# mumianyuxin/M3DSSD

Hardware: AMD Instinct MI355X
Metric: images/sec at 1280x384 bs=8, 1/2/4/8 MI355X; 3D-box Linf vs ref (higher is better)
Workload: dtype f32; 1 GPU; BASELINE.json configs[1]: full M3d_inference_align (DLA-34 + DCNv2 align + ANAB) forward + decode + top-3000 + NMS, bs=8/GPU, 1280x384, fp32, random-init synthetic weights and frames; per_gpu_batch=8, global_batch=8, parallelism=dp1 (batch sharded, 1 all-gather of [B,40,14] detections)

## Files before the change

### include/m3dssd_hip.h

```cpp
#ifndef M3DSSD_HIP_H
#define M3DSSD_HIP_H

#include <stdint.h>

#ifdef __cplusplus
extern "C" {
#endif

typedef void *m3d_stream_t;

enum {
    M3D_OK = 0,
    M3D_E_ARG = -1,
    M3D_E_HIP = -2,
    M3D_E_WORKSPACE = -3
};

const char *m3d_last_error(void);
#define M3D_ABI_VERSION 5
int m3d_abi_version(void);
const char *m3d_source_hashes(void);

typedef struct m3d_conv_desc {
    const float *in;
// ... 9 lines not shown
    int out_nchw;
    long long out_img_stride;
    const float *scale;
    const float *shift;
    const float *res;
    int res_cs;
    int res_mode;
    int act;
    int sigmoid_from;
    const float *dcn_offmask;
    int dcn_om_cs;
    float *splitk_ws;
    long long splitk_ws_bytes;
} m3d_conv_desc;

int m3d_conv2d_forward(const m3d_conv_desc *d, m3d_stream_t stream);
int m3d_conv2d_splitk_plan(const m3d_conv_desc *d, int *splits, long long *ws_bytes);

int m3d_conv_wave_applicable(const m3d_conv_desc *d);
int m3d_conv_wave_splitk_plan(const m3d_conv_desc *d, int *splits, long long *ws_bytes);
int m3d_conv_wave_forward(const m3d_conv_desc *d, m3d_stream_t stream);
int m3d_conv_wave_forward_wgsplit(const m3d_conv_desc *d, m3d_stream_t stream);
int m3d_conv_wave_wgsplit_width(const m3d_conv_desc *d, int *slices, int *width);

int m3d_wino_conv3x3_forward(const m3d_conv_desc *d, m3d_stream_t stream);
int m3d_wino_conv3x3_variant(const m3d_conv_desc *d);
int m3d_wino_conv3x3_splitk_plan(const m3d_conv_desc *d, int *splits, long long *ws_bytes);
int m3d_wino_conv3x3_forward_ex(const m3d_conv_desc *d, int variant, m3d_stream_t stream);
int m3d_wino44_applicable(const m3d_conv_desc *d);
int m3d_wino44_conv3x3_forward(const m3d_conv_desc *d, m3d_stream_t stream);
int m3d_wino44_conv3x3_forward_ex(const m3d_conv_desc *d, int nb, m3d_stream_t stream);
int m3d_wino44_kpair(const m3d_conv_desc *d);
int m3d_wino44_splitk_plan(const m3d_conv_desc *d, int *splits, long long *ws_bytes);
int m3d_wino44_conv3x3_forward_touch(const m3d_conv_desc *d, int nb, const void *touch, long long touch_bytes, m3d_stream_t stream);

int m3d_cache_touch(const void *p, long long bytes, m3d_stream_t stream);
int m3d_upload_indirect(const void *const *src_slot, void *dst, long long bytes, m3d_stream_t stream);

int m3d_conv2d_tile(const m3d_conv_desc *d, int *bm, int *bn, int *bk, int *grid);

typedef struct m3d_conv_bf16_desc {
    const void *in;
    int in_cs;
    int N, H, W, Cin;
    const void *wgt;
    long long wgt_img_stride;
// ... 346 lines not shown
                            long long box_img_stride, m3d_stream_t stream);

int m3d_anab_pool_partial(const float *kv, int kv_cs, const float *s, int s_cs, const int *items, int n_items,
                          const int *bin_scale, int n_bins, float *partial, int max_slots, int B, int H, int W,
                          int C, m3d_stream_t stream);
int m3d_anab_pool_finish(const float *partial, const int *bin_slots, const float *bin_inv_area, int n_bins,
                         int max_slots, int Ck, int Cv, float *khat, int keys_pad, int ck_pad, float *vhatT,
                         int B, int frag, m3d_stream_t stream);
long long m3d_anab_pool_nested_scratch_bytes(int B, int C);
int m3d_anab_pool_nested(const float *kv, int kv_cs, const float *s, int s_cs, int B, int H, int W, int Ck, int Cv,
                         float *scratch, float *khat, int keys_pad, int ck_pad, float *vhatT, int frag, m3d_stream_t stream);
int m3d_anab_pool_nested_bf16(const void *kv, int kv_cs, const float *s, int s_cs, int B, int H, int W, int Ck, int Cv,
                              float *scratch, float *khat, int keys_pad, int ck_pad, float *vhatT, int frag, m3d_stream_t stream);
int m3d_anab_pool_nested_bf16_ex(const void *kv, int kv_cs, const float *s, int s_cs, int B, int H, int W, int Ck, int Cv,
                                 float *scratch, float *khat, int keys_pad, int ck_pad, float *vhatT, int frag,
                                 void *khat16, void *vhat16, m3d_stream_t stream);
int m3d_anab_attend_f32(const float *q, int q_cs, const float *khat, int k_cs, const float *vhatT, int B, int HW, int Ck,
                        int keys, int keys_pad, int Cv, const float *res, int res_cs, int res_mode, const float *scale,
                        const float *shift, int act, float *out, int out_cs, m3d_stream_t stream);
int m3d_anab_attend_f32_rows(const float *q, int q_cs, const float *khat, int k_cs, const float *vhatT, int B, int HW, int Ck,
                             int keys, int keys_pad, int Cv, const float *res, int res_cs, int res_mode, const float *scale,
                             const float *shift, int act, float *out, int out_cs, const int *rows, const int *n_rows,
                             m3d_stream_t stream);
long long m3d_anab_attention_workspace_bytes(int B, int H, int W, int Ck, int Cv, int backward);
int m3d_anab_attention_forward(const float *q, const float *k, const float *v, const float *g, float *out, int B, int H, int W, int Ck,
                               int Cv, int q_cs, int k_cs, int v_cs, int g_cs, int out_cs, void *workspace, long long workspace_bytes,
                               m3d_stream_t stream);
int m3d_anab_attention_backward(const float *q, const float *k, const float *v, const float *g, const float *grad_out, float *grad_q,
                                float *grad_k, float *grad_v, float *grad_g, int B, int H, int W, int Ck, int Cv, int q_cs, int k_cs,
                                int v_cs, int g_cs, int go_cs, int gq_cs, int gk_cs, int gv_cs, int gg_cs, void *workspace,
                                long long workspace_bytes, m3d_stream_t stream);
long long m3d_anab_attention_workspace_bytes_bf16(int B, int H, int W, int Ck, int Cv, int backward);
int m3d_anab_attention_forward_bf16(const void *q, const void *k, const void *v, const void *g, void *out, int B, int H, int W, int Ck,
                                    int Cv, int q_cs, int k_cs, int v_cs, int g_cs, int out_cs, void *workspace,
                                    long long workspace_bytes, m3d_stream_t stream);
int m3d_anab_attention_backward_bf16(const void *q, const void *k, const void *v, const void *g, const void *grad_out, void *grad_q,
                                     void *grad_k, void *grad_v, void *grad_g, int B, int H, int W, int Ck, int Cv, int q_cs, int k_cs,
                                     int v_cs, int g_cs, int go_cs, int gq_cs, int gk_cs, int gv_cs, int gg_cs, void *workspace,
                                     long long workspace_bytes, m3d_stream_t stream);
int m3d_softmax_rows(float *x, int rows, int valid, int cs, m3d_stream_t stream);

int m3d_bundle_outputs(const float *cls_planar, const float *box_planar, float *cls, float *prob, float *bbox_2d,
                       float *bbox_3d, unsigned int *score_bits, int B, int A, int HW, m3d_stream_t stream);
int m3d_score_keys_planar(const float *cls_planar, unsigned int *score_bits, int B, int A, int HW, m3d_stream_t stream);
long long m3d_topk_decode_workspace_bytes(int B, int R);
int m3d_topk_decode(const unsigned int *score_bits, const float *prob, const float *bbox_2d, const float *bbox_3d,
// ... 75 lines not shown
```

### m3dssd_amd/csrc/anab_attend.hip

```cpp
#include <stdlib.h>

#include "common.h"

#define AF_CV 128
#define AF_KT 32
#define AF_VROW (AF_KT * 4 + 16)

struct AnabF32Args {
    const float *q, *khat, *vhat, *res, *scale, *shift;
    float *out;
    int q_cs, k_cs, HW, Ck, keys, keys_pad, res_cs, out_cs, res_mode, act;
};

template <int CK, int NSPLIT>
__device__ __forceinline__ void anab_attend_f32_body(const AnabF32Args &a, const int img, const int mq, const bool store)
{
    constexpr int KROW = CK * 4 + 16;
    constexpr int NS4 = CK / 8;
    __shared__ __attribute__((aligned(16))) unsigned char lds[AF_KT * KROW + AF_CV * AF_VROW];
    unsigned char *Ks = lds, *Vs = lds + AF_KT * KROW;
    const int tid = threadIdx.x, lane = tid & 63;
    const int l31 = lane & 31, lh = lane >> 5;

    f32x4 qf[NS4];
// ... 199 lines not shown
    }
    M3D_LAUNCH_CHECK();
    return M3D_OK;
}

extern "C" int m3d_anab_attend_f32(const float *q, int q_cs, const float *khat, int k_cs, const float *vhatT, int B, int HW, int Ck,
                                   int keys, int keys_pad, int Cv, const float *res, int res_cs, int res_mode, const float *scale,
                                   const float *shift, int act, float *out, int out_cs, m3d_stream_t stream)
{
    return anab_attend_f32_launch(q, q_cs, khat, k_cs, vhatT, B, HW, Ck, keys, keys_pad, Cv, res, res_cs, res_mode, scale, shift, act,
                                  out, out_cs, nullptr, nullptr, stream);
}

extern "C" int m3d_anab_attend_f32_rows(const float *q, int q_cs, const float *khat, int k_cs, const float *vhatT, int B, int HW, int Ck,
                                        int keys, int keys_pad, int Cv, const float *res, int res_cs, int res_mode,
                                        const float *scale, const float *shift, int act, float *out, int out_cs, const int *rows,
                                        const int *n_rows, m3d_stream_t stream)
{
    M3D_REQUIRE(rows && n_rows, "anab_attend_f32_rows: null row list");
    M3D_REQUIRE((long long)B * HW < 0x7FFFFFFFLL - 64, "anab_attend_f32_rows: too many pixels");
    return anab_attend_f32_launch(q, q_cs, khat, k_cs, vhatT, B, HW, Ck, keys, keys_pad, Cv, res, res_cs, res_mode, scale, shift, act,
                                  out, out_cs, rows, n_rows, stream);
}
```

### m3dssd_amd/csrc/dcn_wave.hip

```cpp

#include <type_traits>

#include "common.h"

struct ConvWaveArgs {
    const float *in, *wfrag, *scale, *shift, *res, *om;
    float *out;
    int in_cs, out_cs, res_cs, om_cs;
    int H, W, Cin, Ho, Wo, HoWo, Cout;
    int kh, kw, stride, pad, dil;
    int M, KG, tiles_n;
    int act, res_mode, sigmoid_from;
    int vec_out;
    long long w_img_stride;
    unsigned in_bytes, out_bytes, res_bytes, w_bytes;
    float *ws;
    int splits, ss_per, base_waves;
    unsigned ws_bytes;
#ifdef CONV_TRACE
    long long *trace;
#endif
};


#ifdef CONV_TRACE
static long long *g_conv_trace = nullptr;
extern "C" void m3d_conv_wave_set_trace(void *buf) { g_conv_trace = (long long *)buf; }
static int g_conv_variant = 0;
extern "C" void m3d_conv_wave_set_variant(int v) { g_conv_variant = v; }
#define TRACE_INIT() long long *trp = (a.trace && threadIdx.x < 64) ? a.trace + (size_t)blockIdx.x * 128 : nullptr; int tri = 0
#define TRACE() do { if (trp && lane == 0 && tri < 128) trp[tri++] = __builtin_readcyclecounter(); } while (0)
#else
#define TRACE_INIT()
#define TRACE()
#endif

template <bool DEFORM, int NT, int NCQ = 4, int WPE = (DEFORM ? 2 : 3), int S = 1>
__global__ __launch_bounds__(64 * S) __attribute__((amdgpu_waves_per_eu(WPE))) void conv_wave_kernel(const ConvWaveArgs a)
{
    __shared__ __attribute__((aligned(16))) float tileS[S * 32 * 32];
    __shared__ __attribute__((aligned(16))) float tapst[(DEFORM ? 9 : 1) * 32 * 8];
    const int lane = threadIdx.x & 63, l31 = lane & 31, h = lane >> 5;
    const int wv = S > 1 ? __builtin_amdgcn_readfirstlane((int)threadIdx.x >> 6) : 0;
    float *const tileA = tileS + wv * 1024;
    const int gp = lane >> 3, gc = lane & 7;
    TRACE_INIT();
    TRACE();
    int blk;
    {
        const int nblk = gridDim.x, bid = blockIdx.x;
        const int q = nblk >> 3, r = nblk & 7, xcd = bid & 7, loc = bid >> 3;
        blk = (xcd < r ? xcd * (q + 1) : r * (q + 1) + (xcd - r) * q) + loc;
    }
    int split = wv;
    if (S == 1 && a.splits > 1) {
        split = blk / a.base_waves;
        blk -= split * a.base_waves;
    }
    const int bm = blk / a.tiles_n, bn = blk - bm * a.tiles_n;
    const int m0 = bm * 32;
    const int KK = a.kh * a.kw, C32 = a.Cin / 32;
    const bool idle = S > 1 && wv >= a.splits;
    const int ss0 = idle ? 0 : split * a.ss_per, ss1 = idle ? 0 : min(KK * C32, ss0 + a.ss_per);

    const __amdgpu_buffer_rsrc_t rin = make_rsrc(a.in, a.in_bytes);
    const __amdgpu_buffer_rsrc_t rw =
        make_rsrc(a.wfrag + (size_t)(m0 / a.HoWo) * a.w_img_stride + (size_t)bn * NT * a.KG * 256, a.w_bytes);
    const unsigned wlane = (unsigned)lane * 16u;
    const unsigned wstride = (unsigned)a.KG * 1024u;

    int o_pix = 0, o_hi0 = 0, o_wi0 = 0;
    bool o_valid = false;
    int o_inv = -1;
    const float *o_om = a.om;
    int g_pix[4], g_hi0[4], g_wi0[4];
    bool g_valid[4];
    {
        const int m = m0 + l31;
        o_valid = m < a.M;
        o_inv = sign_smear(a.M - 1 - m);
        const int mm = o_valid ? m : 0;
        const int n = mm / a.HoWo, rem = mm - n * a.HoWo;
        const int ho = rem / a.Wo, wo = rem - ho * a.Wo;
        o_pix = n * a.H * a.W;
        o_hi0 = ho * a.stride - a.pad;
        o_wi0 = wo * a.stride - a.pad;
        if (DEFORM) o_om = a.om + (size_t)mm * a.om_cs;
    }
    if constexpr (!DEFORM) {
#pragma unroll
        for (int g = 0; g < 4; ++g) {
            const int m = m0 + 8 * g + gp;
            g_valid[g] = m < a.M;
            const int mm = g_valid[g] ? m : 0;
            const int n = mm / a.HoWo, rem = mm - n * a.HoWo;
            const int ho = rem / a.Wo, wo = rem - ho * a.Wo;
            g_pix[g] = n * a.H * a.W;
            g_hi0[g] = ho * a.stride - a.pad;
            g_wi0[g] = wo * a.stride - a.pad;
        }
    }

    unsigned doff[4][DEFORM ? 4 : 1];
    float bw[DEFORM ? 4 : 1][4];
    if constexpr (DEFORM) {
        constexpr int TPW = (9 + S - 1) / S;
        float raws[TPW][3];
#pragma unroll
        for (int i = 0; i < TPW; ++i) {
            const int tp = min(wv + i * S, KK - 1);
            raws[i][0] = o_om[2 * tp];
            raws[i][1] = o_om[2 * tp + 1];
            raws[i][2] = o_om[2 * KK + tp];
        }
#pragma unroll
        for (int i = 0; i < TPW; ++i) {
            const int t = wv + i * S;
// ... 200 lines not shown
                    const float *p = &tileS[px[q] * 32 + 4 * c4];
                    f32x4 v = *reinterpret_cast<const f32x4 *>(p);
#pragma unroll
                    for (int s = 1; s < S; ++s)
                        if (s < a.splits) v = v + *reinterpret_cast<const f32x4 *>(p + s * 1024);
                    v = conv_epi_affine(v, scv[nt], shv[nt], a.res ? rv[q] : v, a.res != nullptr, a.res_mode);
                    v = conv_epi_act4(v, c, a.sigmoid_from, tile_sig, slope);
                    if (full) {
                        __builtin_amdgcn_raw_buffer_store_b128(__builtin_bit_cast(u32x4, v), rout, oq[q] + (unsigned)c * 4u, 0, 0);
                    } else {
#pragma unroll
                        for (int e = 0; e < 4; ++e) {
                            const float pe = v[e];
                            __builtin_amdgcn_raw_buffer_store_b32(__builtin_bit_cast(unsigned, pe), rout,
                                                                  c + e < a.Cout ? oq[q] + (unsigned)(c + e) * 4u : M3D_BUF_OOB, 0, 0);
                        }
                    }
                }
            }
        }
        TRACE();
        return;
    }
    if (a.splits > 1) {
        const __amdgpu_buffer_rsrc_t rws = make_rsrc(a.ws, a.ws_bytes);
        const unsigned sbase = (unsigned)split * (unsigned)a.M;
        const unsigned cpad = (unsigned)(a.tiles_n * 32 * NT);
#pragma unroll
        for (int nt = 0; nt < NT; ++nt) {
            const unsigned co = (unsigned)(n0 + nt * 32 + l31);
#pragma unroll
            for (int r = 0; r < 16; ++r) {
                const int m = mb + (r & 3) + 8 * (r >> 2);
                const unsigned oo = m < a.M ? ((sbase + (unsigned)m) * cpad + co) * 4u : M3D_BUF_OOB;
                const float pv = acc[nt][r];
                __builtin_amdgcn_raw_buffer_store_b32(__builtin_bit_cast(unsigned, pv), rws, oo, 0, 0);
            }
        }
        return;
    }
    if (a.vec_out) {
        const float slope = a.act == 1 ? M3D_LEAKY_SLOPE : 1.f;
        const int pr = lane >> 3, c4 = lane & 7;
        unsigned oq[4], rq[4];
#pragma unroll
        for (int q = 0; q < 4; ++q) {
            const int m = m0 + pr + 8 * q;
            oq[q] = m < a.M ? (unsigned)m * (unsigned)a.out_cs * 4u : M3D_BUF_OOB;
            rq[q] = m < a.M ? (unsigned)m * (unsigned)a.res_cs * 4u : M3D_BUF_OOB;
        }
        f32x4 scv[NT], shv[NT];
#pragma unroll
        for (int nt = 0; nt < NT; ++nt) {
            const int c = n0 + nt * 32 + 4 * c4;
            scv[nt] = f32x4{1.f, 1.f, 1.f, 1.f};
            shv[nt] = f32x4{0.f, 0.f, 0.f, 0.f};
            if (c + 3 < a.Cout) {
                if (a.scale) scv[nt] = *reinterpret_cast<const f32x4 *>(a.scale + c);
                if (a.shift) shv[nt] = *reinterpret_cast<const f32x4 *>(a.shift + c);
            } else {
#pragma unroll
                for (int e = 0; e < 4; ++e)
                    if (c + e < a.Cout) {
                        if (a.scale) scv[nt][e] = a.scale[c + e];
                        if (a.shift) shv[nt][e] = a.shift[c + e];
                    }
            }
        }
#pragma unroll
        for (int nt = 0; nt < NT; ++nt) {
            const int c = n0 + nt * 32 + 4 * c4;
            f32x4 rv[4];
// ... 13 lines not shown
#pragma unroll
            for (int r = 0; r < 16; ++r) tileA[((r & 3) + 8 * (r >> 2) + 4 * h) * 32 + l31] = acc[nt][r];
            const bool tile_sig = a.sigmoid_from >= 0 && n0 + nt * 32 + 31 >= a.sigmoid_from;
#pragma unroll
            for (int q = 0; q < 4; ++q) {
                f32x4 v = *reinterpret_cast<const f32x4 *>(&tileA[(pr + 8 * q) * 32 + 4 * c4]);
                v = conv_epi_affine(v, scv[nt], shv[nt], a.res ? rv[q] : v, a.res != nullptr, a.res_mode);
                v = conv_epi_act4(v, c, a.sigmoid_from, tile_sig, slope);
                if (c + 3 < a.Cout) {
                    __builtin_amdgcn_raw_buffer_store_b128(__builtin_bit_cast(u32x4, v), rout, oq[q] + (unsigned)c * 4u, 0, 0);
                } else {
#pragma unroll
                    for (int e = 0; e < 4; ++e) {
                        const float pe = v[e];
                        __builtin_amdgcn_raw_buffer_store_b32(__builtin_bit_cast(unsigned, pe), rout,
                                                              c + e < a.Cout ? oq[q] + (unsigned)(c + e) * 4u : M3D_BUF_OOB, 0, 0);
                    }
                }
            }
        }
        TRACE();
        return;
    }
#pragma unroll
    for (int nt = 0; nt < NT; ++nt) {
        const int co = n0 + nt * 32 + l31;
        const bool cok = co < a.Cout;
        const float sc = (cok && a.scale) ? a.scale[co] : 1.f;
        const float sh = (cok && a.shift) ? a.shift[co] : 0.f;
        float rv[16];
        if (a.res) {
#pragma unroll
            for (int r = 0; r < 16; ++r) {
                const int m = mb + (r & 3) + 8 * (r >> 2);
                const unsigned ro = (cok && m < a.M) ? ((unsigned)m * (unsigned)a.res_cs + (unsigned)co) * 4u : M3D_BUF_OOB;
                rv[r] = __builtin_bit_cast(float, __builtin_amdgcn_raw_buffer_load_b32(rres, ro, 0, 0));
            }
        }
#pragma unroll
        for (int r = 0; r < 16; ++r) {
            const int m = mb + (r & 3) + 8 * (r >> 2);
            float v = conv_epi_affine(acc[nt][r], sc, sh, a.res ? rv[r] : 0.f, a.res != nullptr, a.res_mode);
            v = conv_epi_act(v, a.sigmoid_from >= 0 && co >= a.sigmoid_from, a.act == 1 ? M3D_LEAKY_SLOPE : 1.f);
            const unsigned oo = (cok && m < a.M) ? ((unsigned)m * (unsigned)a.out_cs + (unsigned)co) * 4u : M3D_BUF_OOB;
            __builtin_amdgcn_raw_buffer_store_b32(__builtin_bit_cast(unsigned, v), rout, oo, 0, 0);
        }
    }
    TRACE();
}

static int conv_wave_plan(const m3d_conv_desc *d, bool enforce_min, int *splits, int *ss_per, bool allow32 = false)
{
    *splits = 1;
    *ss_per = d->kh * d->kw * (d->Cin / 32);
    if (d->out_nchw) return 0;
    if (d->dcn_offmask && d->kh * d->kw > 9) return 0;
    if (d->Cin % 32 != 0 || d->Cout_pad % 32 != 0) return 0;
    if (d->Cout_pad % 64 != 0 && (!allow32 || d->dcn_offmask || d->wgt_img_stride)) return 0;
    const int cw = d->Cout_pad % 128 == 0 ? 128 : (d->Cout_pad % 64 == 0 ? 64 : 32);
    if (d->wgt_img_stride && (d->Ho * d->Wo) % 32 != 0) return 0;
    const long long M = (long long)d->N * d->Ho * d->Wo;
    const long long base = ((M + 31) / 32) * (d->Cout_pad / cw);
    if (base >= (1ll << 28)) return 0;
    static const int wave_min = m3d_env_int("M3D_CONV_WAVE_MIN", 900);
    static const int dcn_min = m3d_env_int("M3D_DCN_WAVE_MIN", 1500);
    static const int splitk = m3d_env_int("M3D_CONV_WAVE_SPLITK", 1);
    const long long need = d->dcn_offmask ? dcn_min : wave_min;
// ... 21 lines not shown
{
    M3D_REQUIRE(d && splits && ws_bytes, "conv_wave_splitk_plan: null pointer");
    m3d_conv_desc t = *d;
    static float dummy;
    t.splitk_ws = &dummy;
    int p;
    const int waves = conv_wave_plan(&t, true, splits, &p, true);
    if (waves == 0) *splits = 1;
    *ws_bytes = (*splits > 1 && d->Cout_pad % 64 == 0) ? (long long)*splits * d->N * d->Ho * d->Wo * d->Cout_pad * 4 : 0;
    return M3D_OK;
}

template <bool DEFORM, int NT>
static void launch_wgsplit(const ConvWaveArgs &a, int S, int wgs, hipStream_t stream)
{
    constexpr int WPE = DEFORM ? 2 : 3;
    switch (S) {
    case 2: hipLaunchKernelGGL((conv_wave_kernel<DEFORM, NT, 4, WPE, 2>), dim3(wgs), dim3(128), 0, stream, a); break;
    case 4: hipLaunchKernelGGL((conv_wave_kernel<DEFORM, NT, 4, WPE, 4>), dim3(wgs), dim3(256), 0, stream, a); break;
    default: hipLaunchKernelGGL((conv_wave_kernel<DEFORM, NT, 4, WPE, 8>), dim3(wgs), dim3(512), 0, stream, a); break;
    }
}

static int conv_wave_run(const m3d_conv_desc *d_, hipStream_t stream, bool wgsplit)
{
    M3D_REQUIRE(d_ && d_->in && d_->wgt && d_->out, "conv_wave: null pointer");
    m3d_conv_desc dd = *d_;
    static float dummy;
    if (wgsplit) { dd.splitk_ws = &dummy; dd.splitk_ws_bytes = 0; }
    const m3d_conv_desc *d = &dd;
    int splits = 1, ss_per = 0;
    const int waves = conv_wave_plan(d, false, &splits, &ss_per, wgsplit);
    M3D_REQUIRE(waves > 0, "conv_wave: needs Cin %% 32 == 0, Cout_pad %% 64 == 0 (%% 32: plain, shared weights, wgsplit entry), NHWC output, "
                           "Ho*Wo %% 32 == 0 with per-image weights");
    const int ho = (d->H + 2 * d->pad - (d->dil * (d->kh - 1) + 1)) / d->stride + 1;
    const int wo = (d->W + 2 * d->pad - (d->dil * (d->kw - 1) + 1)) / d->stride + 1;
    M3D_REQUIRE(ho == d->Ho && wo == d->Wo, "conv_wave: Ho/Wo mismatch");
    M3D_REQUIRE(d->in_cs % 32 == 0 && d->in_cs >= d->Cin && ((uintptr_t)d->in & 127) == 0 && ((uintptr_t)d->wgt & 15) == 0,
                "conv_wave: the input view must be 128-byte aligned with in_cs %% 32 == 0");
    const long long M = (long long)d->N * d->Ho * d->Wo;
    M3D_REQUIRE(!d->wgt_img_stride || (d->wgt_img_stride % 4 == 0 && d->stride == 1 && d->Ho == d->H && d->Wo == d->W),
                "conv_wave: per-image weights need an image-aligned 16-byte stride and a same-size output");
    M3D_REQUIRE((long long)d->N * d->H * d->W * d->in_cs * 4 < (1ll << 31) && M * d->out_cs * 4 < (1ll << 31) &&
                M * d->res_cs * 4 < (1ll << 31) && (long long)d->Cout_pad * d->kh * d->kw * d->Cin * 4 < (1ll << 31),
                "conv_wave: views must be < 2 GiB");
    ConvWaveArgs a;
    a.in = d->in; a.wfrag = d->wgt; a.scale = d->scale; a.shift = d->shift; a.res = d->res; a.om = d->dcn_offmask;
    a.out = d->out;
    a.in_cs = d->in_cs; a.out_cs = d->out_cs; a.res_cs = d->res_cs; a.om_cs = d->dcn_om_cs;
    a.H = d->H; a.W = d->W; a.Cin = d->Cin; a.Ho = d->Ho; a.Wo = d->Wo; a.HoWo = d->Ho * d->Wo; a.Cout = d->Cout;
    a.kh = d->kh; a.kw = d->kw; a.stride = d->stride; a.pad = d->pad; a.dil = d->dil;
    const int cw = d->Cout_pad % 128 == 0 ? 128 : (d->Cout_pad % 64 == 0 ? 64 : 32);
    a.M = (int)M; a.KG = d->kh * d->kw * d->Cin / 8; a.tiles_n = d->Cout_pad / cw;
    a.act = d->act; a.res_mode = d->res_mode; a.sigmoid_from = d->sigmoid_from; a.w_img_stride = d->wgt_img_stride;
    static const int vec_epi = m3d_env_int("M3D_WAVE_VEC_EPILOGUE", 1);
    a.vec_out = vec_epi && d->out_cs % 4 == 0 && ((uintptr_t)d->out & 15) == 0 &&
                (!d->res || (d->res_cs % 4 == 0 && ((uintptr_t)d->res & 15) == 0)) &&
                (!d->scale || ((uintptr_t)d->scale & 15) == 0) && (!d->shift || ((uintptr_t)d->shift & 15) == 0);
    a.in_bytes = (unsigned)((long long)d->N * d->H * d->W * d->in_cs * 4);
    a.out_bytes = (unsigned)(M * d->out_cs * 4);
    a.res_bytes = (unsigned)(M * d->res_cs * 4);
    a.w_bytes = (unsigned)((long long)cw * d->kh * d->kw * d->Cin * 4);
#ifdef CONV_TRACE
    a.trace = g_conv_trace;
#endif
    a.ws = nullptr; a.splits = 1; a.ss_per = ss_per; a.base_waves = waves; a.ws_bytes = 0;
    if (splits > 1 && wgsplit) {
        const int S = splits <= 2 ? 2 : (splits <= 4 ? 4 : 8);
        M3D_REQUIRE(splits <= 8, "conv_wave: %d K slices do not fit a workgroup", splits);
        a.splits = splits; a.base_waves = waves / splits;
        if (cw == 128) {
            if (d->dcn_offmask) launch_wgsplit<true, 4>(a, S, a.base_waves, stream);
            else launch_wgsplit<false, 4>(a, S, a.base_waves, stream);
        } else if (cw == 64) {
            if (d->dcn_offmask) launch_wgsplit<true, 2>(a, S, a.base_waves, stream);
            else launch_wgsplit<false, 2>(a, S, a.base_waves, stream);
        } else {
            launch_wgsplit<false, 1>(a, S, a.base_waves, stream);
        }
        M3D_LAUNCH_CHECK();
        return M3D_OK;
    }
    if (splits > 1) {
        const long long need = (long long)splits * M * d->Cout_pad * 4;
        M3D_REQUIRE(need <= d->splitk_ws_bytes && need < (1ll << 31) && ((uintptr_t)d->splitk_ws & 15) == 0,
                    "conv_wave: split-K workspace too small (%lld bytes, see m3d_conv_wave_splitk_plan), >= 2 GiB or misaligned",
                    d->splitk_ws_bytes);
        a.ws = d->splitk_ws; a.splits = splits; a.base_waves = waves / splits; a.ws_bytes = (unsigned)need;
    }
// ... 15 lines not shown
        else hipLaunchKernelGGL((conv_wave_kernel<false, 4>), dim3(waves), dim3(64), 0, stream, a);
    } else if (cw == 32) {
        hipLaunchKernelGGL((conv_wave_kernel<false, 1>), dim3(waves), dim3(64), 0, stream, a);
    } else {
        if (d->dcn_offmask) hipLaunchKernelGGL((conv_wave_kernel<true, 2>), dim3(waves), dim3(64), 0, stream, a);
        else hipLaunchKernelGGL((conv_wave_kernel<false, 2>), dim3(waves), dim3(64), 0, stream, a);
    }
    M3D_LAUNCH_CHECK();
    if (splits > 1) {
        SplitkReduceArgs r;
        r.ws = a.ws; r.scale = d->scale; r.shift = d->shift; r.res = d->res; r.out = d->out;
        r.M = (int)M; r.Cout = d->Cout; r.Cout_pad = d->Cout_pad; r.splits = splits; r.out_cs = d->out_cs; r.res_cs = d->res_cs;
        r.res_mode = d->res_mode; r.act = d->act; r.sigmoid_from = d->sigmoid_from;
        return m3d_launch_splitk_reduce(r, stream);
    }
    return M3D_OK;
}

extern "C" int m3d_conv_wave_forward(const m3d_conv_desc *d, m3d_stream_t stream)
{
    return conv_wave_run(d, (hipStream_t)stream, false);
}

extern "C" int m3d_conv_wave_wgsplit_width(const m3d_conv_desc *d, int *slices, int *width)
{
    M3D_REQUIRE(d && slices && width, "conv_wave_wgsplit_width: null pointer");
    m3d_conv_desc t = *d;
    static float dummy;
    t.splitk_ws = &dummy;
    int p;
    const int waves = conv_wave_plan(&t, false, slices, &p, true);
    M3D_REQUIRE(waves > 0 && *slices <= 8, "conv_wave_wgsplit_width: the wave kernel does not apply to this descriptor");
    *width = *slices <= 1 ? 1 : (*slices <= 2 ? 2 : (*slices <= 4 ? 4 : 8));
    return M3D_OK;
}

extern "C" int m3d_conv_wave_forward_wgsplit(const m3d_conv_desc *d, m3d_stream_t stream)
{
    return conv_wave_run(d, (hipStream_t)stream, true);
}
```

### m3dssd_amd/engine.py

```python
import collections
import ctypes
import math
import os

import numpy as np
import torch

from . import _hip
from ._hip import ConvDesc, MlpDesc
from .config import model_flags

BN_EPS = 1e-5
SELECT_KEYS = os.environ.get("M3D_SELECT_KEYS", "1") != "0"
SPARSE_HEADS_MAX_FRACTION = 0.5
PSP_SIZES = (1, 4, 8, 16)
BACKBONE_CHANNELS = {"dla34": (16, 32, 64, 128, 256, 512), "dla102": (16, 32, 128, 256, 512, 1024)}
BACKBONE_TREES = {"dla34": ((1, 2, 2, 1), 2, False), "dla102": ((1, 3, 4, 1), 3, True)}
BOX_HEADS = ("bbox_x", "bbox_y", "bbox_w", "bbox_h", "bbox_x3d", "bbox_y3d", "bbox_z3d", "bbox_w3d", "bbox_h3d", "bbox_l3d", "bbox_rY3d")


def _rup(a, b):
    return (a + b - 1) // b * b


# ... 96 lines not shown


def pack_wino44(weight, cout_pad, device):
    g = weight.detach().to("cpu", torch.float64)
    co, ci = g.shape[0], g.shape[1]
    assert g.shape[2:] == (3, 3) and ci % 16 == 0 and cout_pad % 32 == 0 and cout_pad >= co
    u = torch.einsum("ai,ocij,bj->aboc", _WINO44_G, g, _WINO44_G).reshape(36, co, ci)
    if cout_pad != co:
        u = torch.cat([u, u.new_zeros(36, cout_pad - co, ci)], 1)
    u = u.view(36, cout_pad // 32, 2, 16, ci // 16, 4, 4).permute(1, 4, 0, 2, 5, 3, 6).contiguous()
    return u.to(torch.float32).reshape(-1).to(device)


def pack_wino44_c16(weight, device):
    g = weight.detach().to("cpu", torch.float64)
    assert tuple(g.shape) == (16, 16, 3, 3)
    u = torch.einsum("ai,ocij,bj->abco", _WINO44_G, g, _WINO44_G).reshape(36, 4, 4, 16)
    return u.permute(0, 1, 3, 2).contiguous().to(torch.float32).reshape(-1).to(device)


WINO_MIN_BLOCKS = int(os.environ.get("M3D_WINO_MIN_BLOCKS", "128"))
FUSED_ANAB = os.environ.get("M3D_FUSED_ANAB", "1") != "0"
ANAB_ROWS = os.environ.get("M3D_ANAB_ROWS", "1") != "0"
USE_ANAB_WAVE = os.environ.get("M3D_ANAB_WAVE", "1") != "0"
USE_ANAB_NESTED = os.environ.get("M3D_ANAB_NESTED", "1") != "0"
USE_DCN_WAVE = os.environ.get("M3D_DCN_WAVE", "1") != "0"
USE_CONV_WAVE = os.environ.get("M3D_CONV_WAVE", "1") != "0"
USE_CONV_WAVE_WGSPLIT = os.environ.get("M3D_CONV_WAVE_WGSPLIT", "1") != "0"
USE_OFFMASK_WAVE = os.environ.get("M3D_OFFMASK_WAVE", "1") != "0"
USE_WINO = os.environ.get("M3D_WINO", "1") != "0"
USE_WINO44 = os.environ.get("M3D_WINO44", "1") != "0"
WINO44_TOUCH = os.environ.get("M3D_WINO44_TOUCH", "1") != "0"
WINO44_TOUCH_SPAN = int(os.environ.get("M3D_WINO44_TOUCH_SPAN", "2"))
USE_WINO44_SPLITK = os.environ.get("M3D_WINO44_SPLITK", "1") != "0"
W44_SPLIT_NB = 2 if os.environ.get("M3D_W44_SPLIT_NB", "1") == "2" else 1
W44_SPLIT_KPAIR = os.environ.get("M3D_W44_SPLIT_NB", "1") == "3"
WINO44_MIN_WGS = int(os.environ.get("M3D_WINO44_MIN_WGS", "1000000"))
WINO44_MIN_WGS_NB1 = int(os.environ.get("M3D_WINO44_MIN_WGS_NB1", "200"))


class OpCost:

    def __init__(self, hbm_bytes):
        self.hbm_bytes = int(hbm_bytes)


# ... 571 lines not shown
                return heads([(p, x, planar)])
            h1 = self._buf(plan, B, fh, fw, 256)
            self._conv(plan, p + ".0", P[p + ".0"], x, h1, 1, k0 // 2, act=1)
            d, flops = head_desc(p, h1, planar, None)
            ref = ctypes.byref(d)
            plan.ops.append((p + ".mlp", "head_mlp<2,%d>" % d.Cout_pad, flops,
                             lambda st: _hip.check(L.m3d_head_mlp_forward(ref, st)), d))

        head("cls", feats0, (r.cls_pl, NC * A * HW, 0), 3)
        self._rpn_select(plan, r)

        if with_shape:
            om_sa = self._buf(plan, B, fh, fw, 27, 28)
            self._rpn_shape_offsets(plan, r, om_sa, cost=True)
            feats = self._buf(plan, B, fh, fw, c3, name="feats")
            self._conv(plan, "shape_align.dcn", P["shape_align"], feats0, feats, 1, 1, act=0, res=feats0, om=om_sa)
        else:
            feats = plan.named["feats"] = feats0

        def center_align(p, x, kx, ky, mi, out):
            om = self._buf(plan, B, fh, fw, 3, 4)
            self._rpn_center_offsets(plan, r, p, om, kx, ky, mi, cost=True)
            self._conv(plan, p + ".dcn", P[p], x, out, 1, 0, act=0, res=x, om=om)

        z3d_now = [] if with_anab else ["bbox_z3d"]
        if with_center:
            heads([("bbox_x", feats, r.box_planar(0)), ("bbox_y", feats, r.box_planar(1)),
                   ("bbox_x3d", feats, r.box_planar(4)), ("bbox_y3d", feats, r.box_planar(5))])
            f2d = self._buf(plan, B, fh, fw, c3, name="feats_align2d")
            center_align("center_align2d", feats, 0, 1, 0, f2d)
            f3d = self._buf(plan, B, fh, fw, c3, name="feats_align3d")
            center_align("center_align3d", feats, 4, 5, 4, f3d)
            heads([("bbox_w", f2d, r.box_planar(2)), ("bbox_h", f2d, r.box_planar(3))] +
                  [(h, f3d, r.box_planar(self.box_heads.index(h))) for h in z3d_now + ["bbox_w3d", "bbox_h3d", "bbox_l3d", "bbox_rY3d"]])
        else:
            f2d = f3d = plan.named["feats_align2d"] = plan.named["feats_align3d"] = feats
            heads([(h, feats, r.box_planar(k)) for k, h in enumerate(self.box_heads) if h != "bbox_z3d" or not with_anab])

        if with_anab:
            gl = self._buf(plan, B, fh, fw, c3, name="feats_gl", zero=True)
            self._anab_ops(plan, f3d, gl, P["anab.bn.scale"], P["anab.bn.shift"], act=1, res_mode=1)
            head("bbox_z3d", gl, r.box_planar(6))
        else:
            plan.named["feats_gl"] = f3d

        self._rpn_outputs(plan, r)
        self._rpn_tail(plan, r)

    def _rpn_stage(self, plan, B, fh, fw):
        r = _RpnStage(B, self.A, self.NC, fh, fw)
        r.cls_pl = torch.empty(B * r.NC * r.R, device=self.device, dtype=torch.float32)
        r.box_pl = torch.empty(B * 11 * r.R, device=self.device, dtype=torch.float32)
# ... 58 lines not shown
        if not plan.named.get("keys_by_select"):
            return
        L, B, A, HW, R = self.L, r.B, r.A, r.HW, r.R
        t0 = plan.named["score_bits_first_write_op"] + 1
        need = r.need = torch.zeros(B * HW, device=self.device, dtype=torch.uint8)
        rows = r.rows = torch.zeros(B * HW, device=self.device, dtype=torch.int32)
        n_rows = r.n_rows = torch.zeros(1, device=self.device, dtype=torch.int32)
        thresh = torch.zeros(B, device=self.device, dtype=torch.int32)
        nb = L.m3d_need_rows_workspace_bytes(B, HW)
        ws = torch.empty(nb, device=self.device, dtype=torch.uint8)
        plan.keep += [need, rows, n_rows, thresh, ws]
        plan.named.update(need=need, need_rows=rows, n_rows=n_rows, need_thresh=thresh)
        k_pre = plan.named["sparse_k"] = [min(int(self.conf.nms_topN_pre), R)]
        key = r.key
        tail = [("need_rows", "select", 0.0, lambda st: _hip.check(L.m3d_need_rows(
            key.data_ptr(), B, A, HW, int(k_pre[0]), thresh.data_ptr(), need.data_ptr(), rows.data_ptr(), n_rows.data_ptr(),
            ws.data_ptr(), nb, st)), OpCost(B * R * 4 * 4))]
        for i in range(t0, len(plan.ops) - 1):
            op, sparse = plan.ops[i], plan.sparse.get(i)
            tail.append(op if sparse is None else op[:3] + (sparse(r), op[4]))
        plan.tail, plan.tail_start = tail, t0
        self._rpn_post3d(plan, r, t0)

    POST_ROWS_MAX = 4096

    def _rpn_post3d(self, plan, r, t0):
        forms = {i: f for i, f in plan.deferred.items() if i >= t0}
        if not forms or plan.post3d_declined is not None:
            return
        if r.B * int(self.conf.nms_topN_post) > self.POST_ROWS_MAX:
            return
        join = int(plan.named["planar_first_op"])
        reads = {}
        for _, _, rd in forms.values():
            for t in rd:
                reads[t.data_ptr()] = (t, plan.first_write.get(t.data_ptr(), -1))
        if any(w < join for _, w in reads.values()):
            return
        r.post_rows = torch.zeros(r.B * r.HW, device=self.device, dtype=torch.int32)
        r.post_n_rows = torch.zeros(1, device=self.device, dtype=torch.int32)
        plan.keep += [r.post_rows, r.post_n_rows]
        plan.post_rows, plan.post_n_rows = r.post_rows, r.post_n_rows

        def form(op, f):
            factory, name, flops, desc = f
            return (op[0] if name is None else name, op[1], op[2] if flops is None else flops, factory(r),
                    op[4] if desc is None else desc)

        pre = [plan.tail[0]]
        for i in range(t0, len(plan.ops) - 1):
            if i not in forms:
                pre.append(plan.tail[1 + i - t0])
            elif forms[i][0] is not None:
                pre.append(form(plan.ops[i], forms[i][0]))
        plan.tail_pre = pre
        plan.post3d = [form(plan.ops[i], forms[i][1]) for i in sorted(forms)]
        plan.post3d_reads = list(reads.values())

    def _anab_ops(self, plan, x, out, scale, shift, act, res_mode):
        L, P = self.L, self.P
        B, fh, fw = x.n, x.h, x.w
        HW = fh * fw
        ctot, off = self.anab_ctot, self.anab_off
        qkvs = self._buf(plan, B, fh, fw, ctot, _rup(ctot, 32))
        self._conv(plan, "anab.qkvs", P["anab.qkvs"], x, qkvs, 1, 0, act=0, sigmoid_from=off["s"], affine=False)
        n_bins = sum(s * s for s in PSP_SIZES)
        fused = FUSED_ANAB and ((self.cv == 128 and self.ck in (64, 128, 168)) or (self.cv == 256 and self.ck == 168)) \
            and HW % 128 == 0
        wave_ok = (not fused) and USE_ANAB_WAVE and USE_CONV_WAVE and HW % 32 == 0 and self.ck_pad % 32 == 0 and self.cv % 128 == 0
        nw = B * HW // 32
        wave_logits = wave_ok and nw * (_rup(n_bins, 128) // 128) >= 900
        keys_pad = _rup(n_bins, 128) if wave_logits else _rup(n_bins, 32)
        wave_pv = wave_ok and keys_pad % 32 == 0 and nw * (self.cv // 128) >= 900
        frag = (1 if wave_logits else 0) | (2 if wave_pv else 0)
        ckv = self.ck + self.cv
        khat = torch.zeros(B * keys_pad * self.ck_pad, device=self.device, dtype=torch.float32)
        vhatT = torch.zeros(B * self.cv * keys_pad, device=self.device, dtype=torch.float32)
        plan.keep += [khat, vhatT]
        plan.named["anab.khat"], plan.named["anab.vhatT"] = khat, vhatT
        kvv, sv = qkvs.slice(off["k"], ckv), qkvs.slice(off["s"], self.ns)
        self._anab_pool(plan, kvv.ptr, kvv.cs, sv.ptr, sv.cs, B, fh, fw, khat, vhatT, keys_pad, frag, nested=USE_ANAB_NESTED,
                        nested_nbytes=B * HW * (ckv + self.ns) * 4)
        qv = qkvs.slice(off["q"], self.ck_pad)
        if fused:
            rp, rcs = (x.ptr, x.cs) if x is not None else (None, 0)
            sp = scale.data_ptr() if scale is not None else None
            hp = shift.data_ptr() if shift is not None else None

            def attend(fn, *row_list):
                return lambda st: _hip.check(fn(
                    qv.ptr, qv.cs, khat.data_ptr(), self.ck_pad, vhatT.data_ptr(), B, HW, self.ck, n_bins, keys_pad, self.cv, rp,
                    rcs, res_mode, sp, hp, 1 if act else 0, out.ptr, out.cs, *row_list, st))

            self._op(plan, "anab.attend", "anab_attend", attend(L.m3d_anab_attend_f32),
                     flops=2.0 * B * HW * n_bins * (self.ck + self.cv),
                nbytes=B * HW * (self.ck + 3 * self.cv) * 4 + B * keys_pad * (self.ck + self.cv) * 4)
            plan.wrote(out.t)
            if ANAB_ROWS:
                plan.sparse_form(lambda r: attend(L.m3d_anab_attend_f32_rows, r.rows.data_ptr(), r.n_rows.data_ptr()))
                plan.deferred_form(None, (lambda r: attend(L.m3d_anab_attend_f32_rows, r.post_rows.data_ptr(),
                                                           r.post_n_rows.data_ptr()), None, None, None),
                                   [qkvs.t, khat, vhatT] + ([x.t] if x is not None else []))
            else:
                plan.post3d_declined = "the attention runs dense in the tail"
            return
        plan.post3d_declined = "the attention is not the one-launch route"

        def image(v, i):
            return View(v.t, 1, v.h, v.w, v.c, v.cs, v.ptr + 4 * i * v.h * v.w * v.cs)

        def image_gemm(name, inp, outv, wgt, stride, frag, res=None, **kw):
            if frag or HW % 64 == 0:
                self._conv(plan, name, None, inp, outv, 1, 0, res=res, wgt_ptr=wgt.data_ptr(), wgt_img_stride=stride, kh=1, kw=1,
                           wgt_frag=frag, **kw)
                return
            sub = _Plan()
            for i in range(B):
                self._conv(sub, name, None, image(inp, i), image(outv, i), 1, 0, res=None if res is None else image(res, i),
                           wgt_ptr=wgt.data_ptr() + 4 * i * stride, kh=1, kw=1, per_image=True, **kw)
            assert len(sub.ops) == B and len({op[1] for op in sub.ops}) == 1, [op[:2] for op in sub.ops]
            plan.keep += sub.keep
            fns = [op[3] for op in sub.ops]
            plan.ops.append((name, sub.ops[0][1], sum(op[2] for op in sub.ops), lambda st: [fn(st) for fn in fns], sub.ops[0][4]))

        logits = self._buf(plan, B, fh, fw, keys_pad)
# ... 211 lines not shown
```

Baseline: 1642 images/sec.

## Compute ANAB query projection only for post-NMS rows via row-list wave conv

Adds a row-list variant of the wave conv kernel that computes outputs only for listed pixels. The ANAB qkvs 1x1 conv now computes only the key/value/gate channels densely, and the query channels are computed later, only for the rows that survive post-3D selection, right before the sparse attention. This is meant to cut the dense query-projection work across all pixels. An optional row-list path for the center_align2d DCN is added but disabled by default, and that buffer is now zero-initialised.

```diff
diff --git a/include/m3dssd_hip.h b/include/m3dssd_hip.h
--- a/include/m3dssd_hip.h
+++ b/include/m3dssd_hip.h
@@ -55,6 +55,7 @@
 int m3d_conv_wave_forward(const m3d_conv_desc *d, m3d_stream_t stream);
 int m3d_conv_wave_forward_wgsplit(const m3d_conv_desc *d, m3d_stream_t stream);
 int m3d_conv_wave_wgsplit_width(const m3d_conv_desc *d, int *slices, int *width);
+int m3d_conv_wave_forward_rows(const m3d_conv_desc *d, const int *rows, const int *n_rows, int max_rows, m3d_stream_t stream);
 
 int m3d_wino_conv3x3_forward(const m3d_conv_desc *d, m3d_stream_t stream);
 int m3d_wino_conv3x3_variant(const m3d_conv_desc *d);
@@ -447,6 +448,10 @@
                              int keys, int keys_pad, int Cv, const float *res, int res_cs, int res_mode, const float *scale,
                              const float *shift, int act, float *out, int out_cs, const int *rows, const int *n_rows,
                              m3d_stream_t stream);
+int m3d_anab_attend_f32_rows_q(const float *q, int q_cs, const float *khat, int k_cs, const float *vhatT, int B, int HW, int Ck,
+                               int keys, int keys_pad, int Cv, const float *res, int res_cs, int res_mode, const float *scale,
+                               const float *shift, int act, float *out, int out_cs, const int *rows, const int *n_rows,
+                               const float *feat, int feat_cs, const float *wq, int max_rows, m3d_stream_t stream);
 long long m3d_anab_attention_workspace_bytes(int B, int H, int W, int Ck, int Cv, int backward);
 int m3d_anab_attention_forward(const float *q, const float *k, const float *v, const float *g, float *out, int B, int H, int W, int Ck,
                                int Cv, int q_cs, int k_cs, int v_cs, int g_cs, int out_cs, void *workspace, long long workspace_bytes,
diff --git a/m3dssd_amd/csrc/anab_attend.hip b/m3dssd_amd/csrc/anab_attend.hip
--- a/m3dssd_amd/csrc/anab_attend.hip
+++ b/m3dssd_amd/csrc/anab_attend.hip
@@ -245,3 +245,24 @@
     return anab_attend_f32_launch(q, q_cs, khat, k_cs, vhatT, B, HW, Ck, keys, keys_pad, Cv, res, res_cs, res_mode, scale, shift, act,
                                   out, out_cs, rows, n_rows, stream);
 }
+
+extern "C" int m3d_anab_attend_f32_rows_q(const float *q, int q_cs, const float *khat, int k_cs, const float *vhatT, int B, int HW, int Ck,
+                                          int keys, int keys_pad, int Cv, const float *res, int res_cs, int res_mode,
+                                          const float *scale, const float *shift, int act, float *out, int out_cs, const int *rows,
+                                          const int *n_rows, const float *feat, int feat_cs, const float *wq, int max_rows,
+                                          m3d_stream_t stream)
+{
+    M3D_REQUIRE(q && feat && wq && rows && n_rows, "anab_attend_f32_rows_q: null pointer");
+    M3D_REQUIRE(B >= 1 && HW >= 1 && Ck >= 1 && Cv >= 32 && Cv % 32 == 0, "anab_attend_f32_rows_q: bad sizes");
+    const int cq = (Ck + 31) / 32 * 32;
+    M3D_REQUIRE(q_cs >= cq, "anab_attend_f32_rows_q: q_cs = %d holds fewer than the %d query channels written", q_cs, cq);
+    m3d_conv_desc d = {};
+    d.in = feat; d.in_cs = feat_cs; d.N = B; d.H = 1; d.W = HW; d.Cin = Cv;
+    d.wgt = wq; d.Cout = cq; d.Cout_pad = (cq + 127) / 128 * 128;
+    d.kh = d.kw = 1; d.stride = 1; d.pad = 0; d.dil = 1; d.Ho = 1; d.Wo = HW;
+    d.out = const_cast<float *>(q); d.out_cs = q_cs; d.sigmoid_from = -1;
+    const int rc = m3d_conv_wave_forward_rows(&d, rows, n_rows, max_rows, stream);
+    if (rc != M3D_OK) return rc;
+    return m3d_anab_attend_f32_rows(q, q_cs, khat, k_cs, vhatT, B, HW, Ck, keys, keys_pad, Cv, res, res_cs, res_mode, scale, shift,
+                                    act, out, out_cs, rows, n_rows, stream);
+}
diff --git a/m3dssd_amd/csrc/dcn_wave.hip b/m3dssd_amd/csrc/dcn_wave.hip
--- a/m3dssd_amd/csrc/dcn_wave.hip
+++ b/m3dssd_amd/csrc/dcn_wave.hip
@@ -17,6 +17,8 @@
     float *ws;
     int splits, ss_per, base_waves;
     unsigned ws_bytes;
+    const int *rows, *n_rows;
+    int M_map;
 #ifdef CONV_TRACE
     long long *trace;
 #endif
@@ -35,9 +37,10 @@
 #define TRACE()
 #endif
 
-template <bool DEFORM, int NT, int NCQ = 4, int WPE = (DEFORM ? 2 : 3), int S = 1>
+template <bool DEFORM, int NT, int NCQ = 4, int WPE = (DEFORM ? 2 : 3), int S = 1, bool ROWS = false>
 __global__ __launch_bounds__(64 * S) __attribute__((amdgpu_waves_per_eu(WPE))) void conv_wave_kernel(const ConvWaveArgs a)
 {
+    static_assert(!ROWS || S == 1, "the row-list form is unsplit");
     __shared__ __attribute__((aligned(16))) float tileS[S * 32 * 32];
     __shared__ __attribute__((aligned(16))) float tapst[(DEFORM ? 9 : 1) * 32 * 8];
     const int lane = threadIdx.x & 63, l31 = lane & 31, h = lane >> 5;
@@ -47,18 +50,29 @@
     TRACE_INIT();
     TRACE();
     int blk;
-    {
+    if constexpr (ROWS) {
+        blk = blockIdx.x;
+    } else {
         const int nblk = gridDim.x, bid = blockIdx.x;
         const int q = nblk >> 3, r = nblk & 7, xcd = bid & 7, loc = bid >> 3;
         blk = (xcd < r ? xcd * (q + 1) : r * (q + 1) + (xcd - r) * q) + loc;
     }
     int split = wv;
-    if (S == 1 && a.splits > 1) {
+    if (S == 1 && !ROWS && a.splits > 1) {
         split = blk / a.base_waves;
         blk -= split * a.base_waves;
     }
     const int bm = blk / a.tiles_n, bn = blk - bm * a.tiles_n;
     const int m0 = bm * 32;
+    const int M = ROWS ? min(*a.n_rows, a.M) : a.M;
+    if constexpr (ROWS) {
+        if (m0 >= M) return;
+    }
+    auto listed = [&](int m) -> int {
+        const int p = m < M ? a.rows[m] : -1;
+        return (unsigned)p < (unsigned)a.M_map ? p : -1;
+    };
+    (void)M; (void)listed;
     const int KK = a.kh * a.kw, C32 = a.Cin / 32;
     const bool idle = S > 1 && wv >= a.splits;
     const int ss0 = idle ? 0 : split * a.ss_per, ss1 = idle ? 0 : min(KK * C32, ss0 + a.ss_per);
@@ -77,9 +91,17 @@
     bool g_valid[4];
     {
         const int m = m0 + l31;
-        o_valid = m < a.M;
-        o_inv = sign_smear(a.M - 1 - m);
-        const int mm = o_valid ? m : 0;
+        int mm;
+        if constexpr (ROWS) {
+            const int p = listed(m);
+            o_valid = p >= 0;
+            o_inv = sign_smear(p);
+            mm = max(p, 0);
+        } else {
+            o_valid = m < a.M;
+            o_inv = sign_smear(a.M - 1 - m);
+            mm = o_valid ? m : 0;
+        }
         const int n = mm / a.HoWo, rem = mm - n * a.HoWo;
         const int ho = rem / a.Wo, wo = rem - ho * a.Wo;
         o_pix = n * a.H * a.W;
@@ -91,8 +113,15 @@
 #pragma unroll
         for (int g = 0; g < 4; ++g) {
             const int m = m0 + 8 * g + gp;
-            g_valid[g] = m < a.M;
-            const int mm = g_valid[g] ? m : 0;
+            int mm;
+            if constexpr (ROWS) {
+                const int p = listed(m);
+                g_valid[g] = p >= 0;
+                mm = max(p, 0);
+            } else {
+                g_valid[g] = m < a.M;
+                mm = g_valid[g] ? m : 0;
+            }
             const int n = mm / a.HoWo, rem = mm - n * a.HoWo;
             const int ho = rem / a.Wo, wo = rem - ho * a.Wo;
             g_pix[g] = n * a.H * a.W;
@@ -339,7 +368,7 @@
         TRACE();
         return;
     }
-    if (a.splits > 1) {
+    if (!ROWS && a.splits > 1) {
         const __amdgpu_buffer_rsrc_t rws = make_rsrc(a.ws, a.ws_bytes);
         const unsigned sbase = (unsigned)split * (unsigned)a.M;
         const unsigned cpad = (unsigned)(a.tiles_n * 32 * NT);
@@ -363,8 +392,14 @@
 #pragma unroll
         for (int q = 0; q < 4; ++q) {
             const int m = m0 + pr + 8 * q;
-            oq[q] = m < a.M ? (unsigned)m * (unsigned)a.out_cs * 4u : M3D_BUF_OOB;
-            rq[q] = m < a.M ? (unsigned)m * (unsigned)a.res_cs * 4u : M3D_BUF_OOB;
+            if constexpr (ROWS) {
+                const int p = listed(m);
+                oq[q] = p >= 0 ? (unsigned)p * (unsigned)a.out_cs * 4u : M3D_BUF_OOB;
+                rq[q] = p >= 0 ? (unsigned)p * (unsigned)a.res_cs * 4u : M3D_BUF_OOB;
+            } else {
+                oq[q] = m < a.M ? (unsigned)m * (unsigned)a.out_cs * 4u : M3D_BUF_OOB;
+                rq[q] = m < a.M ? (unsigned)m * (unsigned)a.res_cs * 4u : M3D_BUF_OOB;
+            }
         }
         f32x4 scv[NT], shv[NT];
 #pragma unroll
@@ -424,6 +459,11 @@
         TRACE();
         return;
     }
+    int prow[ROWS ? 16 : 1];
+    if constexpr (ROWS) {
+#pragma unroll
+        for (int r = 0; r < 16; ++r) prow[r] = listed(mb + (r & 3) + 8 * (r >> 2));
+    }
 #pragma unroll
     for (int nt = 0; nt < NT; ++nt) {
         const int co = n0 + nt * 32 + l31;
@@ -434,17 +474,21 @@
         if (a.res) {
 #pragma unroll
             for (int r = 0; r < 16; ++r) {
-                const int m = mb + (r & 3) + 8 * (r >> 2);
-                const unsigned ro = (cok && m < a.M) ? ((unsigned)m * (unsigned)a.res_cs + (unsigned)co) * 4u : M3D_BUF_OOB;
+                int m = mb + (r & 3) + 8 * (r >> 2);
+                bool mok = m < a.M;
+                if constexpr (ROWS) { m = prow[r]; mok = m >= 0; }
+                const unsigned ro = (cok && mok) ? ((unsigned)m * (unsigned)a.res_cs + (unsigned)co) * 4u : M3D_BUF_OOB;
                 rv[r] = __builtin_bit_cast(float, __builtin_amdgcn_raw_buffer_load_b32(rres, ro, 0, 0));
             }
         }
 #pragma unroll
         for (int r = 0; r < 16; ++r) {
-            const int m = mb + (r & 3) + 8 * (r >> 2);
+            int m = mb + (r & 3) + 8 * (r >> 2);
+            bool mok = m < a.M;
+            if constexpr (ROWS) { m = prow[r]; mok = m >= 0; }
             float v = conv_epi_affine(acc[nt][r], sc, sh, a.res ? rv[r] : 0.f, a.res != nullptr, a.res_mode);
             v = conv_epi_act(v, a.sigmoid_from >= 0 && co >= a.sigmoid_from, a.act == 1 ? M3D_LEAKY_SLOPE : 1.f);
-            const unsigned oo = (cok && m < a.M) ? ((unsigned)m * (unsigned)a.out_cs + (unsigned)co) * 4u : M3D_BUF_OOB;
+            const unsigned oo = (cok && mok) ? ((unsigned)m * (unsigned)a.out_cs + (unsigned)co) * 4u : M3D_BUF_OOB;
             __builtin_amdgcn_raw_buffer_store_b32(__builtin_bit_cast(unsigned, v), rout, oo, 0, 0);
         }
     }
@@ -512,12 +556,14 @@
     }
 }
 
-static int conv_wave_run(const m3d_conv_desc *d_, hipStream_t stream, bool wgsplit)
+static int conv_wave_run(const m3d_conv_desc *d_, hipStream_t stream, bool wgsplit, const int *rows = nullptr,
+                         const int *n_rows = nullptr, int max_rows = 0)
 {
     M3D_REQUIRE(d_ && d_->in && d_->wgt && d_->out, "conv_wave: null pointer");
     m3d_conv_desc dd = *d_;
     static float dummy;
     if (wgsplit) { dd.splitk_ws = &dummy; dd.splitk_ws_bytes = 0; }
+    if (rows) { dd.splitk_ws = nullptr; dd.splitk_ws_bytes = 0; }
     const m3d_conv_desc *d = &dd;
     int splits = 1, ss_per = 0;
     const int waves = conv_wave_plan(d, false, &splits, &ss_per, wgsplit);
@@ -555,6 +601,19 @@
     a.trace = g_conv_trace;
 #endif
     a.ws = nullptr; a.splits = 1; a.ss_per = ss_per; a.base_waves = waves; a.ws_bytes = 0;
+    a.rows = nullptr; a.n_rows = nullptr; a.M_map = (int)M;
+    if (rows) {
+        M3D_REQUIRE(n_rows && max_rows >= 0 && max_rows <= M, "conv_wave_rows: needs n_rows and 0 <= max_rows <= N*Ho*Wo (got %d)", max_rows);
+        M3D_REQUIRE(cw == 128 && splits == 1 && !d->wgt_img_stride,
+                    "conv_wave_rows: built for Cout_pad %% 128 == 0 and shared weights (a wave's entries may belong to different images)");
+        if (max_rows == 0) return M3D_OK;
+        a.rows = rows; a.n_rows = n_rows; a.M = max_rows;
+        const int grid = (max_rows + 31) / 32 * a.tiles_n;
+        if (d->dcn_offmask) hipLaunchKernelGGL((conv_wave_kernel<true, 4, 4, 2, 1, true>), dim3(grid), dim3(64), 0, stream, a);
+        else hipLaunchKernelGGL((conv_wave_kernel<false, 4, 4, 3, 1, true>), dim3(grid), dim3(64), 0, stream, a);
+        M3D_LAUNCH_CHECK();
+        return M3D_OK;
+    }
     if (splits > 1 && wgsplit) {
         const int S = splits <= 2 ? 2 : (splits <= 4 ? 4 : 8);
         M3D_REQUIRE(splits <= 8, "conv_wave: %d K slices do not fit a workgroup", splits);
@@ -616,6 +675,12 @@
     return conv_wave_run(d, (hipStream_t)stream, false);
 }
 
+extern "C" int m3d_conv_wave_forward_rows(const m3d_conv_desc *d, const int *rows, const int *n_rows, int max_rows, m3d_stream_t stream)
+{
+    M3D_REQUIRE(rows && n_rows, "conv_wave_rows: null row list");
+    return conv_wave_run(d, (hipStream_t)stream, false, rows, n_rows, max_rows);
+}
+
 extern "C" int m3d_conv_wave_wgsplit_width(const m3d_conv_desc *d, int *slices, int *width)
 {
     M3D_REQUIRE(d && slices && width, "conv_wave_wgsplit_width: null pointer");
diff --git a/m3dssd_amd/engine.py b/m3dssd_amd/engine.py
--- a/m3dssd_amd/engine.py
+++ b/m3dssd_amd/engine.py
@@ -142,6 +142,16 @@
 WINO_MIN_BLOCKS = int(os.environ.get("M3D_WINO_MIN_BLOCKS", "128"))
 FUSED_ANAB = os.environ.get("M3D_FUSED_ANAB", "1") != "0"
 ANAB_ROWS = os.environ.get("M3D_ANAB_ROWS", "1") != "0"
+
+
+def anab_q_rows():
+    return os.environ.get("M3D_ANAB_Q_ROWS", "1") != "0"
+
+
+def align2d_rows():
+    return os.environ.get("M3D_ALIGN2D_ROWS", "0") != "0"
+
+
 USE_ANAB_WAVE = os.environ.get("M3D_ANAB_WAVE", "1") != "0"
 USE_ANAB_NESTED = os.environ.get("M3D_ANAB_NESTED", "1") != "0"
 USE_DCN_WAVE = os.environ.get("M3D_DCN_WAVE", "1") != "0"
@@ -759,12 +769,17 @@
             om = self._buf(plan, B, fh, fw, 3, 4)
             self._rpn_center_offsets(plan, r, p, om, kx, ky, mi, cost=True)
             self._conv(plan, p + ".dcn", P[p], x, out, 1, 0, act=0, res=x, om=om)
+            if p == "center_align2d" and align2d_rows() and self._wave_rows_ok(P[p], x):
+                d = desc_with(conv_desc(p + ".dcn", P[p], x, out, 1, 0, act=0, res=x, om=om), wgt=self._rows_frag(p, P[p]).data_ptr())
+                ref, cap = ctypes.byref(d), B * HW
+                plan.deferred_form((lambda r: lambda st: _hip.check(L.m3d_conv_wave_forward_rows(
+                    ref, r.rows.data_ptr(), r.n_rows.data_ptr(), cap, st)), None, None, d), None, [])
 
         z3d_now = [] if with_anab else ["bbox_z3d"]
         if with_center:
             heads([("bbox_x", feats, r.box_planar(0)), ("bbox_y", feats, r.box_planar(1)),
                    ("bbox_x3d", feats, r.box_planar(4)), ("bbox_y3d", feats, r.box_planar(5))])
-            f2d = self._buf(plan, B, fh, fw, c3, name="feats_align2d")
+            f2d = self._buf(plan, B, fh, fw, c3, name="feats_align2d", zero=True)
             center_align("center_align2d", feats, 0, 1, 0, f2d)
             f3d = self._buf(plan, B, fh, fw, c3, name="feats_align3d")
             center_align("center_align3d", feats, 4, 5, 4, f3d)
@@ -869,11 +884,29 @@
         plan.tail, plan.tail_start = tail, t0
         self._rpn_post3d(plan, r, t0)
 
+    def _anab_q_rows(self, plan, i_qkvs, x, qkvs):
+        pc, L = self.P["anab.qkvs"], self.L
+        ctot, off = self.anab_ctot, self.anab_off
+        nkvs = ctot - self.ck_pad
+        if not (anab_q_rows() and self._wave_rows_ok(pc, x) and pc.kh * pc.kw == 1 and x.c == self.cv and off["q"] == 0
+                and off["k"] == self.ck_pad and qkvs.cs >= ctot):
+            return None
+        kvs_pad = _rup(nkvs, 128 if os.environ.get("M3D_ANAB_KVS_TILE", "64") == "128" else 64)
+        rows_pad = max(pc.cout_pad, _rup(self.ck_pad, 128), self.ck_pad + kvs_pad)
+        d = conv_desc("anab.qkvs", pc, x, qkvs.slice(self.ck_pad, nkvs), 1, 0, act=0, sigmoid_from=off["s"] - self.ck_pad,
+                      affine=False, cout=nkvs, cout_pad=kvs_pad)
+        frag = self._rows_frag("anab.qkvs", pc, rows_pad)
+        assert frag.numel() == rows_pad * x.c
+        d = desc_with(d, wgt=frag.data_ptr() + 4 * self.ck_pad * x.c)
+        pre = (lambda r: self._launch(L.m3d_conv_wave_forward, d), None, 2.0 * x.n * x.h * x.w * nkvs * x.c, d)
+        plan.deferred[i_qkvs] = (pre, None, [])
+        return frag.data_ptr()
+
     POST_ROWS_MAX = 4096
 
     def _rpn_post3d(self, plan, r, t0):
         forms = {i: f for i, f in plan.deferred.items() if i >= t0}
-        if not forms or plan.post3d_declined is not None:
+        if not any(f[1] is not None for f in forms.values()) or plan.post3d_declined is not None:
             return
         if r.B * int(self.conf.nms_topN_post) > self.POST_ROWS_MAX:
             return
@@ -901,8 +934,21 @@
             elif forms[i][0] is not None:
                 pre.append(form(plan.ops[i], forms[i][0]))
         plan.tail_pre = pre
-        plan.post3d = [form(plan.ops[i], forms[i][1]) for i in sorted(forms)]
+        plan.post3d = [form(plan.ops[i], forms[i][1]) for i in sorted(forms) if forms[i][1] is not None]
         plan.post3d_reads = list(reads.values())
+
+    def _rows_frag(self, key, pc, rows_pad=None):
+        rows_pad = pc.cout_pad if rows_pad is None else rows_pad
+        if pc._frag is not None and rows_pad == pc.cout_pad:
+            return pc._frag
+        cache = self.__dict__.setdefault("_rows_frags", {})
+        if (key, rows_pad) not in cache:
+            cache[key, rows_pad] = pack_frag(pc.wp.view(pc.cout_pad, pc.kh * pc.kw * pc.cin_pad), rows_pad, self.device)
+        return cache[key, rows_pad]
+
+    def _wave_rows_ok(self, pc, x):
+        return (USE_CONV_WAVE and USE_DCN_WAVE and x.cs % 32 == 0 and x.ptr % 128 == 0 and pc.cin_pad == x.c and x.c % 32 == 0
+                and pc.cout_pad % 128 == 0 and pc.kh * pc.kw <= 9)
 
     def _anab_ops(self, plan, x, out, scale, shift, act, res_mode):
         L, P = self.L, self.P
@@ -911,6 +957,7 @@
         ctot, off = self.anab_ctot, self.anab_off
         qkvs = self._buf(plan, B, fh, fw, ctot, _rup(ctot, 32))
         self._conv(plan, "anab.qkvs", P["anab.qkvs"], x, qkvs, 1, 0, act=0, sigmoid_from=off["s"], affine=False)
+        i_qkvs = len(plan.ops) - 1
         n_bins = sum(s * s for s in PSP_SIZES)
         fused = FUSED_ANAB and ((self.cv == 128 and self.ck in (64, 128, 168)) or (self.cv == 256 and self.ck == 168)) \
             and HW % 128 == 0
@@ -945,9 +992,13 @@
             plan.wrote(out.t)
             if ANAB_ROWS:
                 plan.sparse_form(lambda r: attend(L.m3d_anab_attend_f32_rows, r.rows.data_ptr(), r.n_rows.data_ptr()))
-                plan.deferred_form(None, (lambda r: attend(L.m3d_anab_attend_f32_rows, r.post_rows.data_ptr(),
-                                                           r.post_n_rows.data_ptr()), None, None, None),
-                                   [qkvs.t, khat, vhatT] + ([x.t] if x is not None else []))
+                wq = self._anab_q_rows(plan, i_qkvs, x, qkvs) if x is not None else None
+                if wq is None:
+                    post = lambda r: attend(L.m3d_anab_attend_f32_rows, r.post_rows.data_ptr(), r.post_n_rows.data_ptr())
+                else:
+                    post = lambda r: attend(L.m3d_anab_attend_f32_rows_q, r.post_rows.data_ptr(), r.post_n_rows.data_ptr(),
+                                            x.ptr, x.cs, wq, min(r.B * r.HW, self.POST_ROWS_MAX))
+                plan.deferred_form(None, (post, None, None, None), [qkvs.t, khat, vhatT] + ([x.t] if x is not None else []))
             else:
                 plan.post3d_declined = "the attention runs dense in the tail"
             return
```

After: 1656 images/sec (median of 6 runs). About the same (+0.9%).
